# lab-emi/CleanUMamba

Hardware: AMD Instinct MI355X
Metric: audio samples/sec/node (train step, E8, 10s@16kHz) (higher is better)
Workload: dtype f16

## Files before the change

### cleanumamba_amd/csrc/gemm.hip

```cpp
#include <stdlib.h>
#include <type_traits>
#include "common.h"

namespace cum {

typedef __attribute__((ext_vector_type(8))) __bf16 bf16x8;
typedef __attribute__((ext_vector_type(8))) _Float16 f16x8;
typedef __attribute__((ext_vector_type(4))) float f32x4;
typedef __attribute__((ext_vector_type(4))) unsigned u32x4;

enum { EPI_BIAS = 0, EPI_RELU = 1, EPI_GLU = 2, EPI_MASK = 3, EPI_GLU_BWD = 4 };

struct GemmParams {
  const void *A, *W;
  const float *bias;
  const void *res;
  void *out;
  void *aux;
  const void *aux2;
  int64_t lda, ldw, ldc, ldr, ldz, ldy;
  int gate_only;
  int allow_split_k;
  int mask_bits;
  int M, N, K;
  int pitch, valid;
  int n_store;
  int64_t zero_head, zero_tail;
  int rows_epilogue;
  int group_m;
};

template <typename T>
struct Elem;
template <>
struct Elem<float> {
  static constexpr int EPC = 4;
  static __device__ __forceinline__ float to_f(float v) { return v; }
  static __device__ __forceinline__ float from_f(float v) { return v; }
};
template <>
struct Elem<__bf16> {
  static constexpr int EPC = 8;
  static __device__ __forceinline__ float to_f(__bf16 v) { return (float)v; }
  static __device__ __forceinline__ __bf16 from_f(float v) { return (__bf16)v; }
};

template <>
struct Elem<f16> {
  static constexpr int EPC = 8;
  static __device__ __forceinline__ float to_f(f16 v) { return (float)v; }
  static __device__ __forceinline__ f16 from_f(float v) { return (f16)v; }
};

template <typename T>
__device__ __forceinline__ void store4(T *p, const float (&v)[4]);
template <>
__device__ __forceinline__ void store4<float>(float *p, const float (&v)[4]) {
  *reinterpret_cast<float4 *>(p) = make_float4(v[0], v[1], v[2], v[3]);
}
template <>
__device__ __forceinline__ void store4<__bf16>(__bf16 *p, const float (&v)[4]) {
  typedef __attribute__((ext_vector_type(4))) __bf16 bf16x4;
  bf16x4 o = {(__bf16)v[0], (__bf16)v[1], (__bf16)v[2], (__bf16)v[3]};
  *reinterpret_cast<bf16x4 *>(p) = o;
}
template <>
__device__ __forceinline__ void store4<f16>(f16 *p, const float (&v)[4]) {
  typedef __attribute__((ext_vector_type(4))) _Float16 f16x4;
  f16x4 o = {(f16)v[0], (f16)v[1], (f16)v[2], (f16)v[3]};
  *reinterpret_cast<f16x4 *>(p) = o;
}
template <typename T>
__device__ __forceinline__ void load4(const T *p, float (&v)[4]);
template <>
__device__ __forceinline__ void load4<float>(const float *p, float (&v)[4]) {
  const float4 t = *reinterpret_cast<const float4 *>(p);
  v[0] = t.x; v[1] = t.y; v[2] = t.z; v[3] = t.w;
}
template <>
__device__ __forceinline__ void load4<__bf16>(const __bf16 *p, float (&v)[4]) {
  typedef __attribute__((ext_vector_type(4))) __bf16 bf16x4;
  const bf16x4 t = *reinterpret_cast<const bf16x4 *>(p);
#pragma unroll
  for (int i = 0; i < 4; ++i) v[i] = (float)t[i];
}

template <>
__device__ __forceinline__ void load4<f16>(const f16 *p, float (&v)[4]) {
  typedef __attribute__((ext_vector_type(4))) _Float16 f16x4;
  const f16x4 t = *reinterpret_cast<const f16x4 *>(p);
#pragma unroll
  for (int i = 0; i < 4; ++i) v[i] = (float)t[i];
}

template <typename T>
__device__ __forceinline__ void nt_compute(const uint4 *ldsA, const uint4 *ldsW, f32x4 (&acc)[4][4], int wm, int wn,
                                           int g, int r) {
  if constexpr (sizeof(T) == 2) {
#pragma unroll
    for (int ks = 0; ks < 2; ++ks) {
      uint4 wf[4], af[4];
#pragma unroll
      for (int i = 0; i < 4; ++i) {
        const int wrow = wn * 64 + i * 16 + r;
        const int arow = wm * 64 + i * 16 + r;
        const int cl = ks * 4 + g;
        wf[i] = ldsW[wrow * 8 + (cl ^ (wrow & 7))];
        af[i] = ldsA[arow * 8 + (cl ^ (arow & 7))];
      }
#pragma unroll
      for (int ni = 0; ni < 4; ++ni)
#pragma unroll
        for (int mi = 0; mi < 4; ++mi) {
          if constexpr (__is_same(T, f16))
            acc[ni][mi] = __builtin_amdgcn_mfma_f32_16x16x32_f16(__builtin_bit_cast(f16x8, wf[ni]),
                                                                 __builtin_bit_cast(f16x8, af[mi]), acc[ni][mi], 0, 0, 0);
          else
            acc[ni][mi] = __builtin_amdgcn_mfma_f32_16x16x32_bf16(__builtin_bit_cast(bf16x8, wf[ni]),
                                                                  __builtin_bit_cast(bf16x8, af[mi]), acc[ni][mi], 0, 0, 0);
        }
    }
  } else {
#pragma unroll
    for (int h = 0; h < 2; ++h) {
      float wf[4][4], af[4][4];
#pragma unroll
      for (int i = 0; i < 4; ++i) {
        const int wrow = wn * 64 + i * 16 + r;
        const int arow = wm * 64 + i * 16 + r;
        const int cl = 2 * g + h;
        const uint4 wv = ldsW[wrow * 8 + (cl ^ (wrow & 7))];
        const uint4 av = ldsA[arow * 8 + (cl ^ (arow & 7))];
        wf[i][0] = __builtin_bit_cast(float, wv.x); wf[i][1] = __builtin_bit_cast(float, wv.y);
        wf[i][2] = __builtin_bit_cast(float, wv.z); wf[i][3] = __builtin_bit_cast(float, wv.w);
        af[i][0] = __builtin_bit_cast(float, av.x); af[i][1] = __builtin_bit_cast(float, av.y);
        af[i][2] = __builtin_bit_cast(float, av.z); af[i][3] = __builtin_bit_cast(float, av.w);
      }
#pragma unroll
      for (int s = 0; s < 4; ++s)
#pragma unroll
        for (int ni = 0; ni < 4; ++ni)
#pragma unroll
          for (int mi = 0; mi < 4; ++mi)
            acc[ni][mi] = __builtin_amdgcn_mfma_f32_16x16x4f32(wf[ni][s], af[mi][s], acc[ni][mi], 0, 0, 0);
    }
  }
}

__device__ __forceinline__ void nt_load_bias(const GemmParams &p, int n0, int wn, int g, float (&bv)[4][4]) {
#pragma unroll
  for (int ni = 0; ni < 4; ++ni) {
    const int n = n0 + wn * 64 + ni * 16 + 4 * g;
    float4 t = make_float4(0.f, 0.f, 0.f, 0.f);
    if (p.bias && n + 3 < p.N) t = *reinterpret_cast<const float4 *>(p.bias + n);
    bv[ni][0] = t.x; bv[ni][1] = t.y; bv[ni][2] = t.z; bv[ni][3] = t.w;
  }
}

template <typename T>
struct Raw4;
template <>
struct Raw4<float> {
  float4 v;
  __device__ __forceinline__ void ld(const float *p) { v = *reinterpret_cast<const float4 *>(p); }
  __device__ __forceinline__ void get(float (&o)[4]) const { o[0] = v.x; o[1] = v.y; o[2] = v.z; o[3] = v.w; }
};
template <>
struct Raw4<__bf16> {
  typedef __attribute__((ext_vector_type(4))) __bf16 bf16x4;
  bf16x4 v;
  __device__ __forceinline__ void ld(const __bf16 *p) { v = *reinterpret_cast<const bf16x4 *>(p); }
  __device__ __forceinline__ void get(float (&o)[4]) const {
#pragma unroll
    for (int i = 0; i < 4; ++i) o[i] = (float)v[i];
  }
};

template <>
struct Raw4<f16> {
  typedef __attribute__((ext_vector_type(4))) _Float16 f16x4;
  f16x4 v;
  __device__ __forceinline__ void ld(const f16 *p) { v = *reinterpret_cast<const f16x4 *>(p); }
  __device__ __forceinline__ void get(float (&o)[4]) const {
#pragma unroll
    for (int i = 0; i < 4; ++i) o[i] = (float)v[i];
  }
};

template <typename T, int EPI, int NH = 1, int PIPE = -1>
__device__ __forceinline__ void nt_epilogue(const GemmParams &p, const f32x4 (*accp)[4][4], const float (&bv)[4][4],
                                            int m0, int n0, int wm0, int wn, int g, int r) {
  T *__restrict__ out = static_cast<T *>(p.out);
  T *__restrict__ aux = static_cast<T *>(p.aux);
  const T *__restrict__ res = static_cast<const T *>(p.res);
  const T *__restrict__ aux2 = static_cast<const T *>(p.aux2);
  const int nw0 = n0 + wn * 64;
  constexpr bool kMask = EPI == EPI_MASK;
  constexpr int NL = EPI == EPI_GLU ? 2 : 4;
  struct Slab {
    Raw4<T> r[NL], a[EPI == EPI_GLU_BWD ? 4 : 1], b[EPI == EPI_GLU_BWD ? 4 : 1];
    unsigned char mw[4];
  };
  auto row_of = [&](int sl, bool &live) {
    const int m_raw = m0 + wm0 * 64 + sl * 16 + r;
    live = m_raw < p.M;
    return (int64_t)(live ? m_raw : p.M - 1);
  };
  auto issue = [&](int sl, Slab &s) {
    bool live;
    const int64_t m = row_of(sl, live);
    if constexpr (EPI == EPI_GLU) {
#pragma unroll
      for (int pi = 0; pi < 2; ++pi) {
        const int oc = nw0 / 2 + pi * 16 + 4 * g;
        if (res) s.r[pi].ld(res + m * p.ldr + (oc < p.n_store ? oc : 0));
      }
    } else if constexpr (EPI == EPI_GLU_BWD) {
#pragma unroll
      for (int ni = 0; ni < 4; ++ni) {
        const int n = nw0 + ni * 16 + 4 * g;
        const bool nok = n < p.n_store;
        const int nc = nok ? n : 0;
        const int64_t zc = nok ? 2 * (int64_t)(nw0 + ni * 16) + 4 * g : 4 * g;
        if (res) s.r[ni].ld(res + m * p.ldr + nc);
        if (p.gate_only) {
          s.b[ni].ld(aux + m * p.ldz + nc);
          s.a[ni].ld(aux2 + m * p.ldy + nc);
        } else {
          s.a[ni].ld(aux + m * p.ldz + zc);
          s.b[ni].ld(aux + m * p.ldz + zc + 16);
        }
      }
    } else {
#pragma unroll
      for (int ni = 0; ni < 4; ++ni) {
        const int n = nw0 + ni * 16 + 4 * g;
        if (kMask && p.mask_bits) {
          s.mw[ni] = reinterpret_cast<const unsigned char *>(p.res)[(m * p.ldr + (n < p.n_store ? n : 0)) >> 2];
        } else if (kMask || res) {
          s.r[ni].ld(res + m * p.ldr + (n < p.n_store ? n : 0));
        }
      }
    }
  };
  auto finish = [&](int sl, const Slab &s) {
    const f32x4 (&acc)[4][4] = accp[sl / 4];
    const int mi = sl % 4;
    bool live;
    const int64_t m = row_of(sl, live);
    const bool real = live && (m % p.pitch) < p.valid;
    if constexpr (EPI == EPI_GLU) {
#pragma unroll
      for (int pi = 0; pi < 2; ++pi) {
        const int na = nw0 + (2 * pi) * 16 + 4 * g;
        const int nb = na + 16;
        const int oc = nw0 / 2 + pi * 16 + 4 * g;
        float a[4], b[4], o[4];
#pragma unroll
        for (int j = 0; j < 4; ++j) {
          a[j] = acc[2 * pi][mi][j] + bv[2 * pi][j];
          b[j] = acc[2 * pi + 1][mi][j] + bv[2 * pi + 1][j];
          o[j] = real ? a[j] * sigmoidf_(b[j]) : 0.f;
        }
        if (aux && live && na < p.N) {
          if (p.gate_only) {
            store4<T>(aux + m * p.ldz + oc, b);
          } else {
            store4<T>(aux + m * p.ldz + na, a);
            store4<T>(aux + m * p.ldz + nb, b);
          }
        }
        if (res) {
          float rr[4];
          s.r[pi].get(rr);
#pragma unroll
          for (int j = 0; j < 4; ++j) o[j] = real ? o[j] + rr[j] : 0.f;
        }
        if (live && oc < p.n_store && na < p.N) store4<T>(out + m * p.ldc + oc, o);
      }
    } else if constexpr (EPI == EPI_GLU_BWD) {
#pragma unroll
      for (int ni = 0; ni < 4; ++ni) {
        const int n = nw0 + ni * 16 + 4 * g;
        const int64_t zc = 2 * (int64_t)(nw0 + ni * 16) + 4 * g;
        float d[4], a[4], b[4], da[4], db[4];
#pragma unroll
        for (int j = 0; j < 4; ++j) d[j] = acc[ni][mi][j];
        if (res) {
          float rr[4];
          s.r[ni].get(rr);
#pragma unroll
          for (int j = 0; j < 4; ++j) d[j] += rr[j];
        }
        s.a[ni].get(a);
        s.b[ni].get(b);
#pragma unroll
        for (int j = 0; j < 4; ++j) {
          const float sg = sigmoidf_(b[j]);
          const float dj = real ? d[j] : 0.f;
          da[j] = dj * sg;
          db[j] = p.gate_only ? dj * a[j] * (1.f - sg) : dj * a[j] * sg * (1.f - sg);
        }
        if (live && n < p.n_store) {
          store4<T>(out + m * p.ldc + zc, da);
          store4<T>(out + m * p.ldc + zc + 16, db);
        }
      }
    } else {
#pragma unroll
      for (int ni = 0; ni < 4; ++ni) {
        const int n = nw0 + ni * 16 + 4 * g;
        const bool on = live && n < p.n_store;
        float v[4], rr[4] = {0.f, 0.f, 0.f, 0.f};
#pragma unroll
        for (int j = 0; j < 4; ++j) {
          v[j] = acc[ni][mi][j] + bv[ni][j];
          if (EPI == EPI_RELU) v[j] = fmaxf(v[j], 0.f);
          v[j] = real ? v[j] : 0.f;
        }
        if (kMask && p.mask_bits) {
          const unsigned nib = s.mw[ni];
#pragma unroll
          for (int j = 0; j < 4; ++j) rr[j] = (nib >> j) & 1u ? 1.f : 0.f;
        } else if (kMask || res) {
          s.r[ni].get(rr);
        }
        if (aux) {
          if (!kMask && p.mask_bits) {
            unsigned w = 0;
#pragma unroll
            for (int j = 0; j < 4; ++j) w |= (v[j] > 0.f ? 1u : 0u) << j;
            if (on) reinterpret_cast<unsigned char *>(p.aux)[(m * p.ldz + n) >> 2] = (unsigned char)w;
          } else if (on) {
// ... 1094 lines not shown
               : "+a"(acc[7][0]), "+a"(acc[7][1]), "+a"(acc[7][2]), "+a"(acc[7][3]), "+a"(acc[7][4]), "+a"(acc[7][5]),
                 "+a"(acc[7][6]), "+a"(acc[7][7]) : : "memory");
#pragma unroll
  for (int h = 0; h < 2; ++h) {
    float bv[4][4];
    nt_load_bias(p, n0, 2 * wc + h, g, bv);
    f32x4 part[2][4][4];
#pragma unroll
    for (int hh = 0; hh < 2; ++hh)
#pragma unroll
      for (int ni = 0; ni < 4; ++ni)
#pragma unroll
        for (int mi = 0; mi < 4; ++mi) part[hh][ni][mi] = acc[4 * h + ni][4 * hh + mi];
    nt_epilogue_any<T, EPI, 2, 1>(p, part, bv, m0, n0, 2 * wr, 2 * wc + h, lane,
                                  reinterpret_cast<unsigned char *>(lds_all) + wave * nt_rows_lds(EPI));
  }
}
#endif

template <typename T, int EPI>
__global__ __launch_bounds__(256) void gemm_nt_splitk_kernel(const GemmParams p) {
  constexpr int EPC = Elem<T>::EPC, BK = 8 * EPC;
  constexpr int WSTG = 128 * 8;
  __shared__ uint4 lds_all[4 * 2 * WSTG];
  const int tid = threadIdx.x, lane = tid & 63;
  const int wave = uniform(tid >> 6);
  const int g = lane >> 4, r = lane & 15;
  const int NB = (p.N + 63) / 64;
  const int m0 = ((int)blockIdx.x / NB) * 64, n0 = ((int)blockIdx.x % NB) * 64;
  if (blockIdx.x == 0) {
    T *o = static_cast<T *>(p.out);
    T *x = (EPI != EPI_GLU && EPI != EPI_GLU_BWD && !(EPI == EPI_RELU && p.mask_bits)) ? static_cast<T *>(p.aux) : nullptr;
    for (int64_t i = threadIdx.x; i < p.zero_head; i += 256) {
      o[-1 - i] = Elem<T>::from_f(0.f);
      if (x) x[-1 - i] = Elem<T>::from_f(0.f);
    }
    const int64_t tail0 = (int64_t)p.M * p.ldc, tailx = (int64_t)p.M * p.ldz;
    for (int64_t i = threadIdx.x; i < p.zero_tail; i += 256) {
      o[tail0 + i] = Elem<T>::from_f(0.f);
      if (x) x[tailx + i] = Elem<T>::from_f(0.f);
    }
  }
  const T *A = static_cast<const T *>(p.A);
  const T *W = static_cast<const T *>(p.W);
  const T *ga[8], *gw[8];
#pragma unroll
  for (int it = 0; it < 8; ++it) {
    const int row = 8 * it + (lane >> 3), cphys = lane & 7, clog = cphys ^ (row & 7);
    int am = m0 + row, wr = n0 + row;
    am = am < p.M ? am : p.M - 1;
    wr = wr < p.N ? wr : p.N - 1;
    ga[it] = A + (int64_t)am * p.lda + clog * EPC;
    gw[it] = W + (int64_t)wr * p.ldw + clog * EPC;
  }
  typedef __attribute__((address_space(3))) void *lds_ptr;
  typedef const __attribute__((address_space(1))) void *glb_ptr;
  uint4 *mine = lds_all + wave * 2 * WSTG;
  auto issue = [&](int kt, int stage) {
#pragma unroll
    for (int it = 0; it < 8; ++it) {
      __builtin_amdgcn_global_load_lds((glb_ptr)(ga[it] + kt * BK), (lds_ptr)(&mine[stage * WSTG + it * 64]), 16, 0, 0);
      __builtin_amdgcn_global_load_lds((glb_ptr)(gw[it] + kt * BK), (lds_ptr)(&mine[stage * WSTG + 512 + it * 64]), 16, 0, 0);
    }
  };
  f32x4 acc[4][4];
#pragma unroll
  for (int i = 0; i < 4; ++i)
#pragma unroll
    for (int j = 0; j < 4; ++j) acc[i][j] = f32x4{0.f, 0.f, 0.f, 0.f};
  float bv[4][4];
  nt_load_bias(p, n0, 0, g, bv);
  const int nk = p.K / BK;
  int stage = 0;
  if (wave < nk) issue(wave, 0);
  for (int kt = wave; kt < nk; kt += 4) {
    asm volatile("s_waitcnt vmcnt(0)" ::: "memory");
    if (kt + 4 < nk) issue(kt + 4, stage ^ 1);
    nt_compute<T>(mine + stage * WSTG, mine + stage * WSTG + 512, acc, 0, 0, g, r);
    asm volatile("s_waitcnt lgkmcnt(0)" ::: "memory");
    stage ^= 1;
  }
  asm volatile("s_waitcnt vmcnt(0)" ::: "memory");
  f32x4 *park = reinterpret_cast<f32x4 *>(mine);
  if (wave != 0) {
#pragma unroll
    for (int i = 0; i < 4; ++i)
#pragma unroll
      for (int j = 0; j < 4; ++j) park[(i * 4 + j) * 64 + lane] = acc[i][j];
  }
  __syncthreads();
  if (wave != 0) return;
#pragma unroll
  for (int w = 1; w < 4; ++w) {
    const f32x4 *src = reinterpret_cast<const f32x4 *>(lds_all + w * 2 * WSTG);
#pragma unroll
    for (int i = 0; i < 4; ++i)
#pragma unroll
      for (int j = 0; j < 4; ++j) acc[i][j] += src[(i * 4 + j) * 64 + lane];
  }
  nt_epilogue<T, EPI>(p, &acc, bv, m0, n0, 0, 0, g, r);
}

template <typename T>
static int launch_gemm_splitk(const GemmParams &p, int epi, hipStream_t st) {
  dim3 grid(((p.M + 63) / 64) * ((p.N + 63) / 64)), block(256);
  switch (epi) {
    case EPI_BIAS: hipLaunchKernelGGL((gemm_nt_splitk_kernel<T, EPI_BIAS>), grid, block, 0, st, p); break;
    case EPI_RELU: hipLaunchKernelGGL((gemm_nt_splitk_kernel<T, EPI_RELU>), grid, block, 0, st, p); break;
    case EPI_MASK: hipLaunchKernelGGL((gemm_nt_splitk_kernel<T, EPI_MASK>), grid, block, 0, st, p); break;
    case EPI_GLU_BWD: hipLaunchKernelGGL((gemm_nt_splitk_kernel<T, EPI_GLU_BWD>), grid, block, 0, st, p); break;
    default: hipLaunchKernelGGL((gemm_nt_splitk_kernel<T, EPI_GLU>), grid, block, 0, st, p); break;
  }
  CUM_CHECK_LAUNCH();
  return CUM_OK;
}

template <typename T>
__global__ void glu_bwd_kernel(const T *__restrict__ Z, const T *__restrict__ dO, T *__restrict__ dZ, int64_t M,
                               int ngroups, int64_t ldz, int64_t ldo, int n_out) {
  const int64_t total = M * ngroups * 4;
  for (int64_t i = blockIdx.x * (int64_t)blockDim.x + threadIdx.x; i < total; i += (int64_t)gridDim.x * blockDim.x) {
    const int q = i & 3;
    const int64_t t = i >> 2;
    const int grp = t % ngroups;
    const int64_t m = t / ngroups;
    const int oc = grp * 16 + q * 4;
    float a[4], b[4], d[4] = {0.f, 0.f, 0.f, 0.f}, da[4], db[4];
    load4<T>(Z + m * ldz + grp * 32 + q * 4, a);
    load4<T>(Z + m * ldz + grp * 32 + 16 + q * 4, b);
    if (oc < n_out) load4<T>(dO + m * ldo + oc, d);
#pragma unroll
    for (int j = 0; j < 4; ++j) {
      const float s = sigmoidf_(b[j]);
      da[j] = d[j] * s;
      db[j] = d[j] * a[j] * s * (1.f - s);
    }
    store4<T>(dZ + m * ldz + grp * 32 + q * 4, da);
    store4<T>(dZ + m * ldz + grp * 32 + 16 + q * 4, db);
  }
}

template <typename T>
__global__ void glu_bwd_gate_kernel(const T *__restrict__ Bg, const T *__restrict__ Y, const T *__restrict__ dO,
                                    T *__restrict__ dZ, int64_t M, int ngroups, int64_t ldb, int64_t ldy, int64_t ldo,
                                    int64_t ldz, int n_out) {
  const int64_t total = M * ngroups * 4;
  for (int64_t i = blockIdx.x * (int64_t)blockDim.x + threadIdx.x; i < total; i += (int64_t)gridDim.x * blockDim.x) {
    const int q = i & 3;
    const int64_t t = i >> 2;
    const int grp = t % ngroups;
    const int64_t m = t / ngroups;
    const int oc = grp * 16 + q * 4;
    float y[4] = {0.f, 0.f, 0.f, 0.f}, b[4], d[4] = {0.f, 0.f, 0.f, 0.f}, da[4], db[4];
    load4<T>(Bg + m * ldb + oc, b);
    if (oc < n_out) {
      load4<T>(dO + m * ldo + oc, d);
      load4<T>(Y + m * ldy + oc, y);
    }
#pragma unroll
    for (int j = 0; j < 4; ++j) {
      const float s = sigmoidf_(b[j]);
      da[j] = d[j] * s;
      db[j] = d[j] * y[j] * (1.f - s);
    }
    store4<T>(dZ + m * ldz + grp * 32 + q * 4, da);
    store4<T>(dZ + m * ldz + grp * 32 + 16 + q * 4, db);
  }
}

template <typename T>
__global__ void relu_bwd_kernel(const T *__restrict__ Y, const T *__restrict__ dO, T *__restrict__ dZ, int64_t M,
                                int ncol4, int64_t ldy, int64_t ldo, int64_t ldz, int64_t zero_head, int64_t zero_tail) {
  if (blockIdx.x == 0) {
    for (int64_t i = threadIdx.x; i < zero_head; i += blockDim.x) dZ[-1 - i] = Elem<T>::from_f(0.f);
    for (int64_t i = threadIdx.x; i < zero_tail; i += blockDim.x) dZ[M * ldz + i] = Elem<T>::from_f(0.f);
  }
  const int64_t total = M * ncol4;
  for (int64_t i = blockIdx.x * (int64_t)blockDim.x + threadIdx.x; i < total; i += (int64_t)gridDim.x * blockDim.x) {
    const int c = (i % ncol4) * 4;
    const int64_t m = i / ncol4;
    float y[4], d[4];
    load4<T>(Y + m * ldy + c, y);
    load4<T>(dO + m * ldo + c, d);
#pragma unroll
    for (int j = 0; j < 4; ++j) d[j] = y[j] > 0.f ? d[j] : 0.f;
    store4<T>(dZ + m * ldz + c, d);
  }
}

template <typename T>
__global__ void colsum_stage1(const T *__restrict__ X, int64_t M, int n, int64_t ld, int rows_per_block,
                              float *__restrict__ part) {
  const int c = blockIdx.x * blockDim.x + threadIdx.x;
  if (c >= n) return;
  const int64_t r0 = (int64_t)blockIdx.y * rows_per_block;
  int64_t r1 = r0 + rows_per_block;
  r1 = r1 < M ? r1 : M;
  float s = 0.f;
  for (int64_t m = r0; m < r1; ++m) s += Elem<T>::to_f(X[m * ld + c]);
  part[(int64_t)blockIdx.y * n + c] = s;
}
__global__ void colsum_stage2(const float *__restrict__ part, int nparts, int n, float *__restrict__ out) {
  const int c = blockIdx.x * blockDim.x + threadIdx.x;
  if (c >= n) return;
  float s = 0.f;
  for (int i = 0; i < nparts; ++i) s += part[(int64_t)i * n + c];
  out[c] = s;
}

#ifdef CUM_AB
template <typename T>
static int launch_gemm_nt8(const GemmParams &p, int epi, hipStream_t st) {
  if constexpr (sizeof(T) == 2) {
    const int NB = (p.N + 255) / 256, MB = (p.M + 255) / 256;
    dim3 grid(8 * NB * ((MB + 7) / 8)), block(512);
    switch (epi) {
      case EPI_BIAS: hipLaunchKernelGGL((gemm_nt8_kernel<T, EPI_BIAS>), grid, block, 0, st, p); break;
      case EPI_RELU: hipLaunchKernelGGL((gemm_nt8_kernel<T, EPI_RELU>), grid, block, 0, st, p); break;
      case EPI_MASK: hipLaunchKernelGGL((gemm_nt8_kernel<T, EPI_MASK>), grid, block, 0, st, p); break;
      case EPI_GLU_BWD: hipLaunchKernelGGL((gemm_nt8_kernel<T, EPI_GLU_BWD>), grid, block, 0, st, p); break;
      default: hipLaunchKernelGGL((gemm_nt8_kernel<T, EPI_GLU>), grid, block, 0, st, p); break;
    }
    CUM_CHECK_LAUNCH();
  }
  return CUM_OK;
}

#endif

template <typename T>
static int launch_gemm_nt9(const GemmParams &p0, int epi, hipStream_t st) {
  if constexpr (sizeof(T) == 2) {
    GemmParams p = p0;
    const int NB = (p.N + 255) / 256, MB = (p.M + 255) / 256;
    dim3 grid(8 * NB * ((MB + 7) / 8)), block(512);
    p.group_m = (int)cum_knob("CUM_NT_GROUPM", NB >= 24 ? 4 : 1);
    if (p.group_m < 1) p.group_m = 1;
#ifdef CUM_AB
#ifdef CUM_NT4_ONLY_BIAS
    if (cum_knob("CUM_NT4", 0) != 0 && epi == EPI_BIAS) {
      hipLaunchKernelGGL((gemm_nt4_kernel<T, EPI_BIAS>), grid, dim3(256), 0, st, p);
      CUM_CHECK_LAUNCH();
      return CUM_OK;
    }
#else
    if (cum_knob("CUM_NT4", 0) != 0) {
      const dim3 b4(256);
      switch (epi) {
        case EPI_BIAS: hipLaunchKernelGGL((gemm_nt4_kernel<T, EPI_BIAS>), grid, b4, 0, st, p); break;
        case EPI_RELU: hipLaunchKernelGGL((gemm_nt4_kernel<T, EPI_RELU>), grid, b4, 0, st, p); break;
        case EPI_MASK: hipLaunchKernelGGL((gemm_nt4_kernel<T, EPI_MASK>), grid, b4, 0, st, p); break;
        case EPI_GLU_BWD: hipLaunchKernelGGL((gemm_nt4_kernel<T, EPI_GLU_BWD>), grid, b4, 0, st, p); break;
        default: hipLaunchKernelGGL((gemm_nt4_kernel<T, EPI_GLU>), grid, b4, 0, st, p); break;
      }
      CUM_CHECK_LAUNCH();
      return CUM_OK;
    }
#endif
#endif
    switch (epi) {
      case EPI_BIAS: hipLaunchKernelGGL((gemm_nt9_kernel<T, EPI_BIAS>), grid, block, 0, st, p); break;
      case EPI_RELU: hipLaunchKernelGGL((gemm_nt9_kernel<T, EPI_RELU>), grid, block, 0, st, p); break;
      case EPI_MASK: hipLaunchKernelGGL((gemm_nt9_kernel<T, EPI_MASK>), grid, block, 0, st, p); break;
      case EPI_GLU_BWD: hipLaunchKernelGGL((gemm_nt9_kernel<T, EPI_GLU_BWD>), grid, block, 0, st, p); break;
      default: hipLaunchKernelGGL((gemm_nt9_kernel<T, EPI_GLU>), grid, block, 0, st, p); break;
    }
    CUM_CHECK_LAUNCH();
  }
  return CUM_OK;
}

template <typename T>
static int launch_gemm_ring(const GemmParams &p, int epi, hipStream_t st) {
  if constexpr (sizeof(T) == 2) {
    const int NB = (p.N + 255) / 256, MB = (p.M + 127) / 128;
    dim3 grid(8 * NB * ((MB + 7) / 8)), block(512);
    switch (epi) {
      case EPI_BIAS: hipLaunchKernelGGL((gemm_nt_ring_kernel<T, EPI_BIAS>), grid, block, 0, st, p); break;
      case EPI_RELU: hipLaunchKernelGGL((gemm_nt_ring_kernel<T, EPI_RELU>), grid, block, 0, st, p); break;
      case EPI_MASK: hipLaunchKernelGGL((gemm_nt_ring_kernel<T, EPI_MASK>), grid, block, 0, st, p); break;
      case EPI_GLU_BWD: hipLaunchKernelGGL((gemm_nt_ring_kernel<T, EPI_GLU_BWD>), grid, block, 0, st, p); break;
      default: hipLaunchKernelGGL((gemm_nt_ring_kernel<T, EPI_GLU>), grid, block, 0, st, p); break;
    }
    CUM_CHECK_LAUNCH();
  }
  return CUM_OK;
}

template <typename T, int BM, int BN>
static int launch_gemm_tile(const GemmParams &p, int epi, hipStream_t st) {
  const int NB = (p.N + BN - 1) / BN, MB = (p.M + BM - 1) / BM;
  dim3 grid(8 * NB * ((MB + 7) / 8)), block(BM * BN / 64);
  switch (epi) {
    case EPI_BIAS: hipLaunchKernelGGL((gemm_nt_kernel<T, EPI_BIAS, BM, BN>), grid, block, 0, st, p); break;
    case EPI_RELU: hipLaunchKernelGGL((gemm_nt_kernel<T, EPI_RELU, BM, BN>), grid, block, 0, st, p); break;
    case EPI_MASK: hipLaunchKernelGGL((gemm_nt_kernel<T, EPI_MASK, BM, BN>), grid, block, 0, st, p); break;
    case EPI_GLU_BWD: hipLaunchKernelGGL((gemm_nt_kernel<T, EPI_GLU_BWD, BM, BN>), grid, block, 0, st, p); break;
    default: hipLaunchKernelGGL((gemm_nt_kernel<T, EPI_GLU, BM, BN>), grid, block, 0, st, p); break;
  }
  CUM_CHECK_LAUNCH();
  return CUM_OK;
}

static int choose_tile(const GemmParams &p, int esz) {
  const int64_t mb256 = (p.M + 255) / 256;
  const int64_t tiles_256x256 = mb256 * ((p.N + 255) / 256), tiles_256x128 = mb256 * ((p.N + 127) / 128);
  int tile = (int)cum_knob("CUM_NT_TILE", 0);
  const int64_t tiles_128 = ((p.M + 127) / 128) * ((p.N + 127) / 128);
  const int bk = esz == 2 ? 64 : 32;
  if ((tile == 64 || (!tile && (p.allow_split_k == 2 || (p.allow_split_k && tiles_128 <= 64)))) && p.K >= 4 * bk) return 64;
  if (tile == 64) tile = 128;
  if (!tile) {
    if (esz == 2 && p.K >= 256 && tiles_256x256 >= 224 && p.N % 256 == 0 &&
        (int64_t)p.N * p.K >= 256 * (int64_t)(p.N + p.K)) tile = 512;
    else if (esz == 4 && p.K >= 256 && tiles_256x128 >= 1024) tile = 256;
    else if (esz == 2 && p.N % 256 == 0 && p.K >= 512 && ((p.M + 127) / 128) * (int64_t)(p.N / 256) <= cum_knob("CUM_NT_RING", 256) &&
             ((p.M + 127) / 128) * (int64_t)(p.N / 256) >= 40)
      tile = 384;
    else tile = 128;
  }
  if (esz == 2) {
#ifndef CUM_AB
    if (tile == 256) tile = 128;
#endif
    return tile;
  }
  return tile == 512 ? 256 : tile;
}

template <typename T>
static int launch_gemm(const GemmParams &p, int epi, hipStream_t st) {
  const int tile = choose_tile(p, (int)sizeof(T));
  if (tile == 64) return launch_gemm_splitk<T>(p, epi, st);
  if constexpr (sizeof(T) == 2) {
    if (tile == 512) {
#ifdef CUM_AB
      if (cum_knob("CUM_NT9", 1) == 0) return launch_gemm_nt8<T>(p, epi, st);
#endif
      return launch_gemm_nt9<T>(p, epi, st);
    }
    if (tile == 384) return launch_gemm_ring<T>(p, epi, st);
#ifdef CUM_AB
    if (tile == 256) return launch_gemm_tile<T, 256, 128>(p, epi, st);
#endif
    return launch_gemm_tile<T, 128, 128>(p, epi, st);
  } else {
    if (tile == 256) return launch_gemm_tile<T, 256, 128>(p, epi, st);
    return launch_gemm_tile<T, 128, 128>(p, epi, st);
  }
}

}

using namespace cum;

extern "C" int cum_gemm_nt(const cum_gemm_desc *d, const void *A, const void *W, const float *bias, const void *res,
                           void *out, void *aux, const void *aux2, void *stream) {
  CUM_REQUIRE(d && A && W && out, "gemm: null argument");
  CUM_REQUIRE(dtype_ok(d->dtype), "gemm: dtype must be CUM_F32, CUM_BF16 or CUM_F16");
  CUM_REQUIRE(d->epilogue >= 0 && d->epilogue <= 4, "gemm: bad epilogue");
  CUM_REQUIRE(d->epilogue != EPI_MASK || res, "gemm: the MASK epilogue needs the gating activation in res");
  CUM_REQUIRE(d->epilogue != EPI_GLU_BWD || (aux && d->zero_head == 0 && d->zero_tail == 0),
              "gemm: the GLU_BWD epilogue needs Z in aux and writes no framing rows");
  const int bk = is16(d->dtype) ? 64 : 32;
  const int epc = is16(d->dtype) ? 8 : 4;
  CUM_REQUIRE(d->M >= 0 && d->N > 0 && d->K > 0 && d->K % bk == 0, "gemm: K must be a positive multiple of the K tile");
  CUM_REQUIRE(d->N % (d->epilogue == 2 ? 32 : 16) == 0, "gemm: N must be a multiple of 16 (32 for GLU)");
  CUM_REQUIRE(d->lda % epc == 0 && d->ldw % epc == 0, "gemm: lda/ldw must keep rows 16-byte aligned");
  CUM_REQUIRE(d->ldc % 4 == 0 && d->ldr % 4 == 0 && d->ldz % 4 == 0 && d->n_store % 4 == 0, "gemm: ldc/ldr/ldz/n_store must be multiples of 4");
  CUM_REQUIRE(d->pitch > 0 && d->valid >= 0 && d->zero_head >= 0 && d->zero_tail >= 0, "gemm: bad pitch/valid/zero ranges");
  CUM_REQUIRE(((uintptr_t)A & 15) == 0 && ((uintptr_t)W & 15) == 0 && ((uintptr_t)bias & 15) == 0,
              "gemm: A, W and bias must be 16-byte aligned");
  if (d->M == 0) return CUM_OK;
  GemmParams p{};
  CUM_REQUIRE(!d->gate_only || d->epilogue == EPI_GLU || (d->epilogue == EPI_GLU_BWD && aux2 && d->ldy % 4 == 0),
              "gemm: gate_only applies to the GLU epilogues; GLU_BWD then needs the saved output in aux2");
  p.A = A; p.W = W; p.bias = bias; p.res = res; p.out = out; p.aux = aux; p.aux2 = aux2;
  p.lda = d->lda; p.ldw = d->ldw; p.ldc = d->ldc; p.ldr = d->ldr; p.ldz = d->ldz; p.ldy = d->ldy;
  p.gate_only = d->gate_only;
  p.mask_bits = d->mask_bits;
  p.allow_split_k = d->allow_split_k;
  CUM_REQUIRE(!d->mask_bits || (d->epilogue == EPI_RELU && aux) || d->epilogue == EPI_MASK,
              "gemm: mask_bits applies to RELU (aux = sign array) and MASK (res = sign array)");
  p.M = d->M; p.N = d->N; p.K = d->K; p.pitch = d->pitch; p.valid = d->valid; p.n_store = d->n_store;
  p.zero_head = d->zero_head; p.zero_tail = d->zero_tail;
  p.rows_epilogue = (int)cum_knob("CUM_NT8_ROWS", 1);
  if (d->dtype == CUM_BF16) return launch_gemm<__bf16>(p, d->epilogue, (hipStream_t)stream);
  if (d->dtype == CUM_F16) return launch_gemm<f16>(p, d->epilogue, (hipStream_t)stream);
  return launch_gemm<float>(p, d->epilogue, (hipStream_t)stream);
}

extern "C" int cum_gemm_nt_tile(const cum_gemm_desc *d) {
  CUM_REQUIRE(d && dtype_ok(d->dtype), "gemm_nt_tile: bad argument");
  GemmParams p{};
  p.M = d->M; p.N = d->N; p.K = d->K; p.allow_split_k = d->allow_split_k;
  return choose_tile(p, is16(d->dtype) ? 2 : 4);
}

extern "C" int cum_glu_bwd_gate(int32_t dtype, int64_t M, int32_t n_groups, int32_t n_out, const void *Bg, int64_t ldb,
                                const void *Y, int64_t ldy, const void *dOut, int64_t ldo, void *dZ, int64_t ldz,
                                void *stream) {
  CUM_REQUIRE(Bg && Y && dOut && dZ && n_groups > 0 && M >= 0, "glu_bwd_gate: bad argument");
  CUM_REQUIRE(ldb % 4 == 0 && ldy % 4 == 0 && ldo % 4 == 0 && ldz % 4 == 0, "glu_bwd_gate: strides must be multiples of 4");
  if (M == 0) return CUM_OK;
  const int64_t total = M * n_groups * 4;
  int blocks = (int)((total + 255) / 256 < 8192 ? (total + 255) / 256 : 8192);
  if (dtype == CUM_BF16)
    hipLaunchKernelGGL(glu_bwd_gate_kernel<__bf16>, dim3(blocks), dim3(256), 0, (hipStream_t)stream, (const __bf16 *)Bg,
                       (const __bf16 *)Y, (const __bf16 *)dOut, (__bf16 *)dZ, M, n_groups, ldb, ldy, ldo, ldz, n_out);
  else if (dtype == CUM_F16)
    hipLaunchKernelGGL(glu_bwd_gate_kernel<f16>, dim3(blocks), dim3(256), 0, (hipStream_t)stream, (const f16 *)Bg,
                       (const f16 *)Y, (const f16 *)dOut, (f16 *)dZ, M, n_groups, ldb, ldy, ldo, ldz, n_out);
  else
    hipLaunchKernelGGL(glu_bwd_gate_kernel<float>, dim3(blocks), dim3(256), 0, (hipStream_t)stream, (const float *)Bg,
                       (const float *)Y, (const float *)dOut, (float *)dZ, M, n_groups, ldb, ldy, ldo, ldz, n_out);
  CUM_CHECK_LAUNCH();
  return CUM_OK;
}

extern "C" int cum_glu_bwd(int32_t dtype, int64_t M, int32_t n_groups, int32_t n_out, const void *Z, int64_t ldz,
                           const void *dOut, int64_t ldo, void *dZ, void *stream) {
  CUM_REQUIRE(Z && dOut && dZ && n_groups > 0 && M >= 0, "glu_bwd: bad argument");
  CUM_REQUIRE(ldz % 4 == 0 && ldo % 4 == 0, "glu_bwd: strides must be multiples of 4");
  if (M == 0) return CUM_OK;
  const int64_t total = M * n_groups * 4;
  int blocks = (int)((total + 255) / 256 < 8192 ? (total + 255) / 256 : 8192);
  if (dtype == CUM_BF16)
    hipLaunchKernelGGL(glu_bwd_kernel<__bf16>, dim3(blocks), dim3(256), 0, (hipStream_t)stream, (const __bf16 *)Z,
                       (const __bf16 *)dOut, (__bf16 *)dZ, M, n_groups, ldz, ldo, n_out);
  else if (dtype == CUM_F16)
    hipLaunchKernelGGL(glu_bwd_kernel<f16>, dim3(blocks), dim3(256), 0, (hipStream_t)stream, (const f16 *)Z,
                       (const f16 *)dOut, (f16 *)dZ, M, n_groups, ldz, ldo, n_out);
  else
    hipLaunchKernelGGL(glu_bwd_kernel<float>, dim3(blocks), dim3(256), 0, (hipStream_t)stream, (const float *)Z,
                       (const float *)dOut, (float *)dZ, M, n_groups, ldz, ldo, n_out);
  CUM_CHECK_LAUNCH();
  return CUM_OK;
}

extern "C" int cum_relu_bwd(int32_t dtype, int64_t M, int32_t n_cols, const void *Y, int64_t ldy, const void *dOut,
                            int64_t ldo, void *dZ, int64_t ldz, int64_t zero_head, int64_t zero_tail, void *stream) {
  CUM_REQUIRE(Y && dOut && dZ && n_cols > 0 && n_cols % 4 == 0 && M >= 0, "relu_bwd: bad argument");
  CUM_REQUIRE(ldy % 4 == 0 && ldo % 4 == 0 && ldz % 4 == 0, "relu_bwd: strides must be multiples of 4");
  if (M == 0) return CUM_OK;
  const int64_t total = M * (n_cols / 4);
  int blocks = (int)((total + 255) / 256 < 8192 ? (total + 255) / 256 : 8192);
  if (dtype == CUM_BF16)
    hipLaunchKernelGGL(relu_bwd_kernel<__bf16>, dim3(blocks), dim3(256), 0, (hipStream_t)stream, (const __bf16 *)Y,
                       (const __bf16 *)dOut, (__bf16 *)dZ, M, n_cols / 4, ldy, ldo, ldz, zero_head, zero_tail);
  else if (dtype == CUM_F16)
    hipLaunchKernelGGL(relu_bwd_kernel<f16>, dim3(blocks), dim3(256), 0, (hipStream_t)stream, (const f16 *)Y,
                       (const f16 *)dOut, (f16 *)dZ, M, n_cols / 4, ldy, ldo, ldz, zero_head, zero_tail);
  else
    hipLaunchKernelGGL(relu_bwd_kernel<float>, dim3(blocks), dim3(256), 0, (hipStream_t)stream, (const float *)Y,
                       (const float *)dOut, (float *)dZ, M, n_cols / 4, ldy, ldo, ldz, zero_head, zero_tail);
  CUM_CHECK_LAUNCH();
  return CUM_OK;
}

extern "C" int64_t cum_colsum_workspace_elems(int64_t M, int32_t n_cols) {
  const int64_t parts = (M + 1023) / 1024;
  return parts * n_cols;
}

extern "C" int cum_colsum(int32_t dtype, int64_t M, int32_t n_cols, const void *X, int64_t ld, float *out,
                          float *workspace, void *stream) {
  CUM_REQUIRE(X && out && workspace && n_cols > 0 && M >= 0, "colsum: bad argument");
  hipStream_t st = (hipStream_t)stream;
  if (M == 0) {
    (void)hipMemsetAsync(out, 0, sizeof(float) * n_cols, st);
    return CUM_OK;
  }
  const int parts = (int)((M + 1023) / 1024);
  dim3 grid((n_cols + 63) / 64, parts), block(64);
  if (dtype == CUM_BF16)
    hipLaunchKernelGGL(colsum_stage1<__bf16>, grid, block, 0, st, (const __bf16 *)X, M, n_cols, ld, 1024, workspace);
  else if (dtype == CUM_F16)
    hipLaunchKernelGGL(colsum_stage1<f16>, grid, block, 0, st, (const f16 *)X, M, n_cols, ld, 1024, workspace);
  else
    hipLaunchKernelGGL(colsum_stage1<float>, grid, block, 0, st, (const float *)X, M, n_cols, ld, 1024, workspace);
  CUM_CHECK_LAUNCH();
  hipLaunchKernelGGL(colsum_stage2, dim3((n_cols + 63) / 64), dim3(64), 0, st, workspace, parts, n_cols, out);
  CUM_CHECK_LAUNCH();
  return CUM_OK;
}
```

Before: 137.3 million.

## Add row-streaming skinny GEMM kernels for narrow-N and short-K 16-bit shapes

Adds a separate kernel file with two specialized NT GEMM paths for 16-bit bias-only epilogues. One handles narrow N (up to 160) with long K: four waves split K, each keeps register-ring prefetched MFMA accumulators, and the partial sums are reduced through LDS. The other handles short K (up to 256): the A rows stay in registers while W tiles are double-buffered through LDS across 256-wide N chunks. The tile chooser sends eligible shapes to these kernels unless a legacy-route bit is set, aiming to avoid the poor occupancy of large-tile kernels on skinny shapes. The cost is more code paths and alignment assumptions on bias and strides.

```diff
diff --git a/cleanumamba_amd/csrc/gemm.hip b/cleanumamba_amd/csrc/gemm.hip
--- a/cleanumamba_amd/csrc/gemm.hip
+++ b/cleanumamba_amd/csrc/gemm.hip
@@ -1,6 +1,7 @@
 #include <stdlib.h>
 #include <type_traits>
 #include "common.h"
+#include "gemm_skinny.h"
 
 namespace cum {
 
@@ -8,27 +9,6 @@
 typedef __attribute__((ext_vector_type(8))) _Float16 f16x8;
 typedef __attribute__((ext_vector_type(4))) float f32x4;
 typedef __attribute__((ext_vector_type(4))) unsigned u32x4;
-
-enum { EPI_BIAS = 0, EPI_RELU = 1, EPI_GLU = 2, EPI_MASK = 3, EPI_GLU_BWD = 4 };
-
-struct GemmParams {
-  const void *A, *W;
-  const float *bias;
-  const void *res;
-  void *out;
-  void *aux;
-  const void *aux2;
-  int64_t lda, ldw, ldc, ldr, ldz, ldy;
-  int gate_only;
-  int allow_split_k;
-  int mask_bits;
-  int M, N, K;
-  int pitch, valid;
-  int n_store;
-  int64_t zero_head, zero_tail;
-  int rows_epilogue;
-  int group_m;
-};
 
 template <typename T>
 struct Elem;
@@ -1729,7 +1709,8 @@
   return CUM_OK;
 }
 
-static int choose_tile(const GemmParams &p, int esz) {
+static int choose_tile(const GemmParams &p, int esz, int epi) {
+  if (esz == 2 && !p.legacy_route && rowstream_nt_ok(p, epi, CUM_F16)) return NT_TILE_ROWSTREAM;
   const int64_t mb256 = (p.M + 255) / 256;
   const int64_t tiles_256x256 = mb256 * ((p.N + 255) / 256), tiles_256x128 = mb256 * ((p.N + 127) / 128);
   int tile = (int)cum_knob("CUM_NT_TILE", 0);
@@ -1757,7 +1738,8 @@
 
 template <typename T>
 static int launch_gemm(const GemmParams &p, int epi, hipStream_t st) {
-  const int tile = choose_tile(p, (int)sizeof(T));
+  const int tile = choose_tile(p, (int)sizeof(T), epi);
+  if (tile == NT_TILE_ROWSTREAM) return launch_rowstream_nt(p, __is_same(T, f16) ? CUM_F16 : CUM_BF16, st);
   if (tile == 64) return launch_gemm_splitk<T>(p, epi, st);
   if constexpr (sizeof(T) == 2) {
     if (tile == 512) {
@@ -1806,7 +1788,8 @@
   p.lda = d->lda; p.ldw = d->ldw; p.ldc = d->ldc; p.ldr = d->ldr; p.ldz = d->ldz; p.ldy = d->ldy;
   p.gate_only = d->gate_only;
   p.mask_bits = d->mask_bits;
-  p.allow_split_k = d->allow_split_k;
+  p.allow_split_k = d->allow_split_k & 3;
+  p.legacy_route = d->allow_split_k & 4;
   CUM_REQUIRE(!d->mask_bits || (d->epilogue == EPI_RELU && aux) || d->epilogue == EPI_MASK,
               "gemm: mask_bits applies to RELU (aux = sign array) and MASK (res = sign array)");
   p.M = d->M; p.N = d->N; p.K = d->K; p.pitch = d->pitch; p.valid = d->valid; p.n_store = d->n_store;
@@ -1820,8 +1803,12 @@
 extern "C" int cum_gemm_nt_tile(const cum_gemm_desc *d) {
   CUM_REQUIRE(d && dtype_ok(d->dtype), "gemm_nt_tile: bad argument");
   GemmParams p{};
-  p.M = d->M; p.N = d->N; p.K = d->K; p.allow_split_k = d->allow_split_k;
-  return choose_tile(p, is16(d->dtype) ? 2 : 4);
+  p.M = d->M; p.N = d->N; p.K = d->K; p.allow_split_k = d->allow_split_k & 3;
+  p.legacy_route = d->allow_split_k & 4;
+  p.lda = d->lda; p.ldw = d->ldw; p.ldc = d->ldc; p.ldr = d->ldr; p.ldz = d->ldz; p.ldy = d->ldy;
+  p.gate_only = d->gate_only; p.mask_bits = d->mask_bits;
+  p.pitch = d->pitch; p.valid = d->valid; p.n_store = d->n_store; p.zero_head = d->zero_head; p.zero_tail = d->zero_tail;
+  return choose_tile(p, is16(d->dtype) ? 2 : 4, d->epilogue);
 }
 
 extern "C" int cum_glu_bwd_gate(int32_t dtype, int64_t M, int32_t n_groups, int32_t n_out, const void *Bg, int64_t ldb,
diff --git a/cleanumamba_amd/csrc/gemm_skinny.h b/cleanumamba_amd/csrc/gemm_skinny.h
--- /dev/null
+++ b/cleanumamba_amd/csrc/gemm_skinny.h
@@ -0,0 +1,32 @@
+#pragma once
+#include "common.h"
+
+namespace cum {
+
+enum { EPI_BIAS = 0, EPI_RELU = 1, EPI_GLU = 2, EPI_MASK = 3, EPI_GLU_BWD = 4 };
+
+struct GemmParams {
+  const void *A, *W;
+  const float *bias;
+  const void *res;
+  void *out;
+  void *aux;
+  const void *aux2;
+  int64_t lda, ldw, ldc, ldr, ldz, ldy;
+  int gate_only;
+  int allow_split_k;
+  int mask_bits;
+  int M, N, K;
+  int pitch, valid;
+  int n_store;
+  int64_t zero_head, zero_tail;
+  int rows_epilogue;
+  int group_m;
+  int legacy_route;
+};
+
+constexpr int NT_TILE_ROWSTREAM = 32;
+bool rowstream_nt_ok(const GemmParams &p, int epi, int dtype);
+int launch_rowstream_nt(const GemmParams &p, int dtype, hipStream_t st);
+
+}
diff --git a/cleanumamba_amd/csrc/gemm_skinny.hip b/cleanumamba_amd/csrc/gemm_skinny.hip
--- /dev/null
+++ b/cleanumamba_amd/csrc/gemm_skinny.hip
@@ -0,0 +1,292 @@
+#include "common.h"
+#include "gemm_skinny.h"
+
+namespace cum {
+
+typedef __attribute__((ext_vector_type(8))) __bf16 bf16x8;
+typedef __attribute__((ext_vector_type(8))) _Float16 f16x8;
+typedef __attribute__((ext_vector_type(4))) float f32x4;
+typedef __attribute__((ext_vector_type(4))) unsigned u32x4;
+
+template <typename T>
+__device__ __forceinline__ f32x4 mfma16(u32x4 w, u32x4 a, f32x4 c) {
+  if constexpr (__is_same(T, f16))
+    return __builtin_amdgcn_mfma_f32_16x16x32_f16(__builtin_bit_cast(f16x8, w), __builtin_bit_cast(f16x8, a), c, 0, 0, 0);
+  else
+    return __builtin_amdgcn_mfma_f32_16x16x32_bf16(__builtin_bit_cast(bf16x8, w), __builtin_bit_cast(bf16x8, a), c, 0, 0, 0);
+}
+
+template <typename T>
+__device__ __forceinline__ void unpack8(const u32x4 &v, float (&o)[8]) {
+  typedef __attribute__((ext_vector_type(8))) T tx8;
+  const tx8 t = __builtin_bit_cast(tx8, v);
+#pragma unroll
+  for (int i = 0; i < 8; ++i) o[i] = (float)t[i];
+}
+
+template <typename T, int OFF>
+__device__ __forceinline__ u32x4 pack8(const float (&v)[16]) {
+  typedef __attribute__((ext_vector_type(8))) T tx8;
+  tx8 t;
+#pragma unroll
+  for (int i = 0; i < 8; ++i) t[i] = (T)v[OFF + i];
+  return __builtin_bit_cast(u32x4, t);
+}
+
+__device__ __forceinline__ int xcd_logical_block() {
+  const int per = (int)gridDim.x >> 3;
+  return ((int)blockIdx.x & 7) * per + ((int)blockIdx.x >> 3);
+}
+
+constexpr int RS_BM = 32;
+
+template <typename T, int NT, int RING>
+__global__ __launch_bounds__(256) void gemm_nt_rowstream_kernel(const GemmParams p, int total) {
+  __shared__ f32x4 park[3][2 * NT][64];
+  const int L = xcd_logical_block();
+  if (L >= total) return;
+  const int lane = threadIdx.x & 63, wave = uniform(threadIdx.x >> 6);
+  const int g = lane >> 4, r = lane & 15;
+  const int m0 = L * RS_BM;
+  const int kq = wave * (p.K >> 2);
+  const int nsteps = p.K >> 7;
+  const T *ap[2];
+#pragma unroll
+  for (int mi = 0; mi < 2; ++mi) {
+    int m = m0 + 16 * mi + r;
+    m = m < p.M ? m : p.M - 1;
+    ap[mi] = static_cast<const T *>(p.A) + (int64_t)m * p.lda + kq + 8 * g;
+  }
+  const T *wp = static_cast<const T *>(p.W) + (int64_t)r * p.ldw + kq + 8 * g;
+  const int64_t w16 = 16 * p.ldw;
+
+  u32x4 af[RING][2], wf[RING][NT];
+  f32x4 acc[NT][2];
+#pragma unroll
+  for (int ni = 0; ni < NT; ++ni)
+#pragma unroll
+    for (int mi = 0; mi < 2; ++mi) acc[ni][mi] = f32x4{0.f, 0.f, 0.f, 0.f};
+
+  auto load = [&](int slot, int s) {
+#pragma unroll
+    for (int mi = 0; mi < 2; ++mi) af[slot][mi] = *reinterpret_cast<const u32x4 *>(ap[mi] + 32 * s);
+#pragma unroll
+    for (int ni = 0; ni < NT; ++ni) wf[slot][ni] = *reinterpret_cast<const u32x4 *>(wp + ni * w16 + 32 * s);
+  };
+  auto mma = [&](int slot) {
+#pragma unroll
+    for (int ni = 0; ni < NT; ++ni)
+#pragma unroll
+      for (int mi = 0; mi < 2; ++mi) acc[ni][mi] = mfma16<T>(wf[slot][ni], af[slot][mi], acc[ni][mi]);
+  };
+
+#pragma unroll
+  for (int u = 0; u < RING - 1; ++u) load(u, u);
+  int s0 = 0;
+  for (; s0 + RING < nsteps; s0 += RING) {
+#pragma unroll
+    for (int u = 0; u < RING; ++u) {
+      load((u + RING - 1) % RING, s0 + u + RING - 1);
+      mma(u);
+    }
+  }
+  load(RING - 1, s0 + RING - 1);
+#pragma unroll
+  for (int u = 0; u < RING; ++u) mma(u);
+
+  if (wave != 0) {
+#pragma unroll
+    for (int ni = 0; ni < NT; ++ni)
+#pragma unroll
+      for (int mi = 0; mi < 2; ++mi) park[wave - 1][ni * 2 + mi][lane] = acc[ni][mi];
+  }
+  __syncthreads();
+  if (wave != 0) return;
+#pragma unroll
+  for (int w = 0; w < 3; ++w)
+#pragma unroll
+    for (int ni = 0; ni < NT; ++ni)
+#pragma unroll
+      for (int mi = 0; mi < 2; ++mi) acc[ni][mi] += park[w][ni * 2 + mi][lane];
+
+  typedef __attribute__((ext_vector_type(4))) T tx4;
+  T *out = static_cast<T *>(p.out);
+  const T *res = static_cast<const T *>(p.res);
+  f32x4 bv[NT];
+#pragma unroll
+  for (int ni = 0; ni < NT; ++ni) bv[ni] = f32x4{0.f, 0.f, 0.f, 0.f};
+  if (p.bias) {
+#pragma unroll
+    for (int ni = 0; ni < NT; ++ni) bv[ni] = *reinterpret_cast<const f32x4 *>(p.bias + 16 * ni + 4 * g);
+  }
+#pragma unroll
+  for (int mi = 0; mi < 2; ++mi) {
+    const int m = m0 + 16 * mi + r;
+    const int mc = m < p.M ? m : p.M - 1;
+    tx4 rt[NT];
+#pragma unroll
+    for (int ni = 0; ni < NT; ++ni) rt[ni] = tx4{(T)0.f, (T)0.f, (T)0.f, (T)0.f};
+    if (res) {
+#pragma unroll
+      for (int ni = 0; ni < NT; ++ni) rt[ni] = *reinterpret_cast<const tx4 *>(res + (int64_t)mc * p.ldr + 16 * ni + 4 * g);
+    }
+    if (m < p.M) {
+#pragma unroll
+      for (int ni = 0; ni < NT; ++ni) {
+        tx4 o;
+#pragma unroll
+        for (int j = 0; j < 4; ++j) o[j] = (T)(acc[ni][mi][j] + bv[ni][j] + (float)rt[ni][j]);
+        *reinterpret_cast<tx4 *>(out + (int64_t)m * p.ldc + 16 * ni + 4 * g) = o;
+      }
+    }
+  }
+}
+
+constexpr int SK_BM = 64;
+constexpr int SK_BN = 256;
+
+template <typename T, int KS>
+__global__ __launch_bounds__(256) void gemm_nt_rowstream_shortk_kernel(const GemmParams p, int MB, int total) {
+  constexpr int CPR = 4 * KS;
+  constexpr int ROWB = 64 * KS + 16;
+  __shared__ __attribute__((aligned(16))) unsigned char lds[2][64 * ROWB];
+  const int L = xcd_logical_block();
+  if (L >= total) return;
+  const int tid = threadIdx.x, lane = tid & 63, wave = uniform(tid >> 6);
+  const int g = lane >> 4, r = lane & 15;
+  const int nch = L / MB, mb = L - nch * MB;
+  const int nbase = nch * SK_BN;
+  int ngroups = (p.N - nbase) >> 6;
+  ngroups = ngroups < SK_BN / 64 ? ngroups : SK_BN / 64;
+  const int m = mb * SK_BM + 16 * wave + r;
+  const bool live = m < p.M;
+  const int mc = live ? m : p.M - 1;
+
+  u32x4 af[KS];
+  {
+    const T *a = static_cast<const T *>(p.A) + (int64_t)mc * p.lda + 8 * g;
+#pragma unroll
+    for (int ks = 0; ks < KS; ++ks) af[ks] = *reinterpret_cast<const u32x4 *>(a + 32 * ks);
+  }
+
+  const T *W = static_cast<const T *>(p.W);
+  int64_t wsrc[KS];
+  int wdst[KS];
+#pragma unroll
+  for (int i = 0; i < KS; ++i) {
+    const int c = tid + 256 * i, q = c / CPR, ch = c - q * CPR;
+    const int t = q >> 4, rr = q & 15;
+    wsrc[i] = (int64_t)(16 * (rr >> 2) + 4 * t + (rr & 3)) * p.ldw + 8 * ch;
+    wdst[i] = q * ROWB + 16 * ch;
+  }
+  u32x4 wreg[KS];
+#define CUM_SK_FETCH(gi)                                                                                      \
+  _Pragma("unroll") for (int i = 0; i < KS; ++i)                                                              \
+    wreg[i] = *reinterpret_cast<const u32x4 *>(W + (int64_t)(nbase + 64 * (gi)) * p.ldw + wsrc[i])
+#define CUM_SK_STAGE(buf)                                                                                     \
+  _Pragma("unroll") for (int i = 0; i < KS; ++i) *reinterpret_cast<u32x4 *>(&lds[buf][wdst[i]]) = wreg[i]
+
+  T *out = static_cast<T *>(p.out) + (int64_t)mc * p.ldc + nbase + 16 * g;
+  const T *res = p.res ? static_cast<const T *>(p.res) + (int64_t)mc * p.ldr + nbase + 16 * g : nullptr;
+
+  CUM_SK_FETCH(0);
+  CUM_SK_STAGE(0);
+  __syncthreads();
+  for (int gi = 0; gi < ngroups; ++gi) {
+    const int buf = gi & 1;
+    const bool more = gi + 1 < ngroups;
+    if (more) { CUM_SK_FETCH(gi + 1); }
+    u32x4 rv0 = {0u, 0u, 0u, 0u}, rv1 = rv0;
+    if (res) {
+      rv0 = *reinterpret_cast<const u32x4 *>(res + 64 * gi);
+      rv1 = *reinterpret_cast<const u32x4 *>(res + 64 * gi + 8);
+    }
+    f32x4 bv[4];
+#pragma unroll
+    for (int q = 0; q < 4; ++q) bv[q] = f32x4{0.f, 0.f, 0.f, 0.f};
+    if (p.bias) {
+#pragma unroll
+      for (int q = 0; q < 4; ++q) bv[q] = *reinterpret_cast<const f32x4 *>(p.bias + nbase + 64 * gi + 16 * g + 4 * q);
+    }
+    float v[16];
+#pragma unroll
+    for (int t = 0; t < 4; ++t) {
+      f32x4 acc = {0.f, 0.f, 0.f, 0.f};
+      const unsigned char *row = &lds[buf][(16 * t + r) * ROWB + 16 * g];
+#pragma unroll
+      for (int ks = 0; ks < KS; ++ks) acc = mfma16<T>(*reinterpret_cast<const u32x4 *>(row + 64 * ks), af[ks], acc);
+#pragma unroll
+      for (int j = 0; j < 4; ++j) v[4 * t + j] = acc[j];
+    }
+#pragma unroll
+    for (int q = 0; q < 16; ++q) v[q] += bv[q >> 2][q & 3];
+    if (res) {
+      float f[8];
+#pragma unroll
+      for (int h = 0; h < 2; ++h) {
+        unpack8<T>(h ? rv1 : rv0, f);
+#pragma unroll
+        for (int j = 0; j < 8; ++j) v[8 * h + j] += f[j];
+      }
+    }
+    if (live) {
+      *reinterpret_cast<u32x4 *>(out + 64 * gi) = pack8<T, 0>(v);
+      *reinterpret_cast<u32x4 *>(out + 64 * gi + 8) = pack8<T, 8>(v);
+    }
+    if (more) { CUM_SK_STAGE(buf ^ 1); }
+    __syncthreads();
+  }
+#undef CUM_SK_FETCH
+#undef CUM_SK_STAGE
+}
+
+bool rowstream_nt_ok(const GemmParams &p, int epi, int dtype) {
+  if (!is16(dtype) || epi != EPI_BIAS || p.aux || p.mask_bits) return false;
+  if (p.pitch <= 0 || p.valid < p.pitch || p.zero_head || p.zero_tail || p.n_store != p.N) return false;
+  if ((p.lda & 7) || (p.ldw & 7)) return false;
+  if (p.N % 32 == 0 && p.N <= 160 && p.K % 1024 == 0) return true;
+  if (p.K <= 256 && p.K % 64 == 0 && p.N % 64 == 0)
+    return (p.ldc & 7) == 0 && ((uintptr_t)p.out & 15) == 0 && (!p.res || ((p.ldr & 7) == 0 && ((uintptr_t)p.res & 15) == 0));
+  return false;
+}
+
+template <typename T, int NT>
+static void launch_long_k(const GemmParams &p, hipStream_t st) {
+  constexpr int RING = NT <= 4 ? 8 : 4;
+  const int total = (p.M + RS_BM - 1) / RS_BM;
+  hipLaunchKernelGGL((gemm_nt_rowstream_kernel<T, NT, RING>), dim3(8 * ((total + 7) / 8)), dim3(256), 0, st, p, total);
+}
+
+template <typename T, int KS>
+static void launch_short_k(const GemmParams &p, hipStream_t st) {
+  const int MB = (p.M + SK_BM - 1) / SK_BM, total = MB * ((p.N + SK_BN - 1) / SK_BN);
+  hipLaunchKernelGGL((gemm_nt_rowstream_shortk_kernel<T, KS>), dim3(8 * ((total + 7) / 8)), dim3(256), 0, st, p, MB, total);
+}
+
+template <typename T>
+static int launch_rowstream_t(const GemmParams &p, hipStream_t st) {
+  if (p.K > 256) {
+    switch (p.N / 16) {
+      case 2: launch_long_k<T, 2>(p, st); break;
+      case 4: launch_long_k<T, 4>(p, st); break;
+      case 6: launch_long_k<T, 6>(p, st); break;
+      case 8: launch_long_k<T, 8>(p, st); break;
+      default: launch_long_k<T, 10>(p, st); break;
+    }
+  } else {
+    switch (p.K / 64) {
+      case 1: launch_short_k<T, 2>(p, st); break;
+      case 2: launch_short_k<T, 4>(p, st); break;
+      case 3: launch_short_k<T, 6>(p, st); break;
+      default: launch_short_k<T, 8>(p, st); break;
+    }
+  }
+  CUM_CHECK_LAUNCH();
+  return CUM_OK;
+}
+
+int launch_rowstream_nt(const GemmParams &p, int dtype, hipStream_t st) {
+  return dtype == CUM_F16 ? launch_rowstream_t<f16>(p, st) : launch_rowstream_t<__bf16>(p, st);
+}
+
+}
```

Measured after the change: 137.0 million. Within noise of the previous version (-0.2%).
